# i-HamidZafar/Federated-Learning-with-MPI

Hardware: AMD Instinct MI355X
Metric: samples/sec/client + rounds-to-target-accuracy, MLP on income data at 1/2/4/8 clients (higher is better)
Workload: dtype bf16

## Files before the change

### fedmi/ops/csrc/fl_device.h

```cpp
#pragma once
#include "fl_common.h"
#include <math.h>


#define FL_STAMP(i)                                                                            \
    do {                                                                                       \
        if (b.dbg != nullptr && threadIdx.x == 0)                                              \
            b.dbg[blockIdx.x * 16 + (i)] = __builtin_amdgcn_s_memrealtime();                   \
    } while (0)

__device__ __forceinline__ void lds_barrier() { asm volatile("s_waitcnt lgkmcnt(0)\n\ts_barrier" ::: "memory"); }

__device__ __forceinline__ void lds_count_arrive(int* cnt) {
    asm volatile("s_waitcnt lgkmcnt(0)" ::: "memory");
    if ((threadIdx.x & 63) == 0) atomicAdd(cnt, 1);
}
__device__ __forceinline__ void lds_count_wait(int* cnt, int target) {
    while (*reinterpret_cast<volatile int*>(cnt) < target) __builtin_amdgcn_s_sleep(1);
    asm volatile("" ::: "memory");
}

__device__ __forceinline__ void slab_store(float* p, float v) {
#if defined(FL_SLAB_CACHED)
    *p = v;
#elif defined(FL_SLAB_NT)
    __builtin_nontemporal_store(v, p);
#else
    __hip_atomic_store(p, v, __ATOMIC_RELAXED, __HIP_MEMORY_SCOPE_AGENT);
#endif
}

__device__ __forceinline__ void slab_store_h(uint16_t* p, float v) {
    const float c = v == v ? fminf(fmaxf(v, -65504.f), 65504.f) : v;
    const _Float16 h = (_Float16)c;
#if defined(FL_SLAB_CACHED)
    *p = *reinterpret_cast<const uint16_t*>(&h);
#elif defined(FL_SLAB_NT)
    __builtin_nontemporal_store(*reinterpret_cast<const uint16_t*>(&h), p);
#else
    __hip_atomic_store(p, *reinterpret_cast<const uint16_t*>(&h), __ATOMIC_RELAXED, __HIP_MEMORY_SCOPE_AGENT);
#endif
}

__device__ __forceinline__ float wave_sum(float v) {
#pragma unroll
    for (int off = 32; off > 0; off >>= 1) v += __shfl_xor(v, off, 64);
    return v;
}

template <int THREADS>
__device__ __forceinline__ float block_sum_ordered(float acc, float* wsum) {
    acc = wave_sum(acc);
    if ((threadIdx.x & 63) == 0) wsum[threadIdx.x >> 6] = acc;
    __syncthreads();
    float ss = 0.f;
#pragma unroll
    for (int k = 0; k < THREADS / 64; ++k) ss = __fadd_rn(ss, wsum[k]);
    return ss;
}


template <typename CM>
__device__ void metrics_from_cm(CM cmv, int C, double out[4]) {
    double total = 0, tp_sum = 0;
    for (int t = 0; t < C; ++t)
        for (int p = 0; p < C; ++p) {
            const double x = cmv(t, p);
            total += x;
            if (t == p) tp_sum += x;
        }
    if (total <= 0) { out[0] = out[1] = out[2] = out[3] = 0; return; }
    double prec = 0, rec = 0, f1 = 0;
    for (int t = 0; t < C; ++t) {
        double support = 0, pred = 0;
        for (int p = 0; p < C; ++p) { support += cmv(t, p); pred += cmv(p, t); }
        const double tp = cmv(t, t);
        const double w = support / total;
        const double pc = pred > 0 ? tp / pred : 0.0;
        const double rc = support > 0 ? tp / support : 0.0;
        const double den = 2 * tp + (pred - tp) + (support - tp);
        const double fc = den > 0 ? 2 * tp / den : 0.0;
        prec += w * pc; rec += w * rc; f1 += w * fc;
    }
    out[0] = tp_sum / total; out[1] = prec; out[2] = rec; out[3] = f1;
}

static __device__ FLState fold_round(const MLPDesc& d, const FLConfig& c, const FLBuffers& b,
                                     const float* tails, int r, FLState S, bool write_hist) {
    const int lane = threadIdx.x & 63;
    if (S.stopped || r < 0 || r < S.finalized) return S;
    {
        const int C = d.dim[d.L];
        double mk[4] = {0, 0, 0, 0};
        double lk = 0;
        if (lane < c.world) {
            const float* cm = tails + lane * c.tail_stride;
            metrics_from_cm([&](int t, int p) { return (double)cm[t * C + p]; }, C, mk);
            lk = (double)cm[C * C];
            if (write_hist && r < c.max_rounds)
                for (int q = 0; q < 4; ++q) b.hist_rank[((size_t)r * c.world + lane) * 4 + q] = mk[q];
        }
        const float* rt = b.rtab + 4 * (size_t)r;
        const uint32_t m_lo = __float_as_uint(rt[2]), m_hi = __float_as_uint(rt[3]);
        const double n_act = (double)rt[1];
        auto sampled = [&](int k) { return ((k < 32 ? (m_lo >> k) : (m_hi >> (k - 32))) & 1u) != 0; };
        double mean[4] = {0, 0, 0, 0};
        double loss = 0;
        for (int k = 0; k < c.world; ++k) {
            const bool in = sampled(k);
            for (int q = 0; q < 4; ++q) {
                const double v = __shfl(mk[q], k, 64);
                if (in) mean[q] += v;
            }
            const double lv = __shfl(lk, k, 64);
            if (in) loss += lv;
        }
        if (lane != 0) return S;
        if (c.metric_mode == 0) {
            for (int q = 0; q < 4; ++q) mean[q] /= n_act;
        } else {
            metrics_from_cm(
                [&](int t, int p) {
                    double x = 0;
                    for (int k = 0; k < c.world; ++k)
// ... 44 lines not shown
```

### fedmi/ops/csrc/fl_kernels.hip

```cpp
#include "fl_common.h"
#include "fl_device.h"
#include "peer_device.h"
#include "fl_philox.h"
#include "fl_layout.h"
#include <math.h>

typedef float f32x4 __attribute__((ext_vector_type(4)));

__device__ __forceinline__ f32x4 mfma_f32(float a, float b, f32x4 c) {
    return __builtin_amdgcn_mfma_f32_16x16x4f32(a, b, c, 0, 0, 0);
}

__device__ __forceinline__ int fl_swz_lg(int lg) { return (lg == 1 || lg == 2) ? 4 : 0; }

__device__ __forceinline__ float4 lds4(const float* p) { return *reinterpret_cast<const float4*>(p); }
__device__ __forceinline__ float f4(const float4& v, int j) {
    return j == 0 ? v.x : (j == 1 ? v.y : (j == 2 ? v.z : v.w));
}

template <int RT, bool ST = false>
__device__ void fwd_layer_mfma(const float* w, int ldw, const float* bias, int K, int N, const float* in,
                               int ld_in, float* out, int ld_out, bool relu) {
    const int wave = threadIdx.x >> 6, lane = threadIdx.x & 63;
    const int lr = lane & 15, lg = lane >> 4;
    const int ntiles = (N + 15) >> 4;
    const int kchunks = (K + 15) >> 4;
    for (int nt = wave; nt < ntiles; nt += FL_WAVES) {
        const int n = nt * 16 + lr;
        const int ck = (4 * lg) ^ fl_swz(lr);
        const float* wr = w + n * ldw + ck;
        const float* ar = in + lr * ld_in + ck;
        f32x4 acc[RT];
#pragma unroll
        for (int rt = 0; rt < RT; ++rt) acc[rt] = (f32x4){0.f, 0.f, 0.f, 0.f};
        float4 bc = lds4(wr), ac[RT];
#pragma unroll
        for (int rt = 0; rt < RT; ++rt) ac[rt] = lds4(ar + rt * 16 * ld_in);
        const int klast = K - 16 * (kchunks - 1);
#pragma unroll ST ? 16 : 1
        for (int q = 0; q < kchunks; ++q) {
            const int qn = (q + 1 < kchunks) ? q + 1 : q;
            const float4 bn = lds4(wr + 16 * qn);
            float4 an[RT];
#pragma unroll
            for (int rt = 0; rt < RT; ++rt) an[rt] = lds4(ar + rt * 16 * ld_in + 16 * qn);
            __builtin_amdgcn_sched_barrier(0);
            const int jmax = (q + 1 < kchunks || klast > 4) ? 4 : klast;
#pragma unroll
            for (int j = 0; j < 4; ++j)
                if (j < jmax)
#pragma unroll
                    for (int rt = 0; rt < RT; ++rt) acc[rt] = mfma_f32(f4(ac[rt], j), f4(bc, j), acc[rt]);
            __builtin_amdgcn_sched_barrier(0);
            bc = bn;
#pragma unroll
            for (int rt = 0; rt < RT; ++rt) ac[rt] = an[rt];
        }
        const float bv = bias[n];
        const int ns = n ^ fl_swz_lg(lg);
#pragma unroll
        for (int rt = 0; rt < RT; ++rt)
#pragma unroll
            for (int j = 0; j < 4; ++j) {
                float v = acc[rt][j] + bv;
                if (relu) v = fmaxf(v, 0.f);
                out[(rt * 16 + lg * 4 + j) * ld_out + ns] = v;
            }
    }
}

template <int RT>
__device__ void fwd_head_valu(const float* w, int ldw, const float* bias, int K, int C, const float* in,
                              int ld_in, float* out, int ld_out) {
    const int R = RT * 16;
    const int nout = R * C;
    int T = FL_THREADS / nout;
    T = T >= 64 ? 64 : (T >= 32 ? 32 : (T >= 16 ? 16 : (T >= 8 ? 8 : (T >= 4 ? 4 : (T >= 2 ? 2 : 1)))));
    const int K16 = (K + 15) & ~15;
    for (int base = 0; base < nout * T; base += FL_THREADS) {
        const int gid = base + threadIdx.x;
        const int o = gid / T, part = gid - o * T;
        const int oc = o < nout ? o : nout - 1;
        const int r = oc / C, c = oc - r * C;
        const float* ar = in + r * ld_in;
        const float* wr = w + c * ldw;
        const int sa = fl_swz(r), sw = fl_swz(c);
        float s0 = 0.f, s1 = 0.f;
        int k = 4 * part;
        for (; k + 4 * T < K16; k += 8 * T) {
            const float4 a0 = lds4(ar + (k ^ sa)), w0 = lds4(wr + (k ^ sw));
            const float4 a1 = lds4(ar + ((k + 4 * T) ^ sa)), w1 = lds4(wr + ((k + 4 * T) ^ sw));
            s0 = fmaf(a0.x, w0.x, s0); s0 = fmaf(a0.y, w0.y, s0); s0 = fmaf(a0.z, w0.z, s0); s0 = fmaf(a0.w, w0.w, s0);
            s1 = fmaf(a1.x, w1.x, s1); s1 = fmaf(a1.y, w1.y, s1); s1 = fmaf(a1.z, w1.z, s1); s1 = fmaf(a1.w, w1.w, s1);
        }
        if (k < K16) {
            const float4 a0 = lds4(ar + (k ^ sa)), w0 = lds4(wr + (k ^ sw));
            s0 = fmaf(a0.x, w0.x, s0); s0 = fmaf(a0.y, w0.y, s0); s0 = fmaf(a0.z, w0.z, s0); s0 = fmaf(a0.w, w0.w, s0);
        }
        float s = s0 + s1;
        for (int off = 1; off < T; off <<= 1) s += __shfl_xor(s, off, 64);
        if (o < nout && part == 0) out[r * ld_out + (c ^ sa)] = s + bias[c];
    }
    const int Cp = (C + 15) & ~15;
    for (int e = threadIdx.x; e < R * (Cp - C); e += FL_THREADS) {
        const int r = e / (Cp - C), c = C + (e - r * (Cp - C));
        out[r * ld_out + (c ^ fl_swz(r))] = 0.f;
    }
}

__device__ __forceinline__ int wgrad_waves_fp32(int K, int N, int l) {
    const int items = l > 0 ? (K + 15) >> 4 : 0;
    const int chunks = (N + 15) >> 4;
    return (items > 0 && chunks >= 4 && 2 * items <= FL_WAVES) ? FL_WAVES - items : FL_WAVES;
}

template <int RT, bool ST = false>
__device__ void dgrad_layer(const float* w, int ldw, int K, int N, const float* dz, int ld_z, const float* act,
                            int ld_a, float* out) {
    const int wave = (FL_WAVES - 1) - (threadIdx.x >> 6), lane = threadIdx.x & 63;
    const int lr = lane & 15, lg = lane >> 4;
    const int itiles = (K + 15) >> 4;
    const int ochunks = (N + 15) >> 4;
    const bool prio = ochunks >= 4 && wave < itiles;
    if (prio) __builtin_amdgcn_s_setprio(2);
    for (int it = wave; it < itiles; it += FL_WAVES) {
        const int i = it * 16 + lr;
        const int is = i ^ fl_swz_lg(lg);
        const float* wc = w + 4 * lg * ldw + is;
        const float* ar = dz + lr * ld_z + ((4 * lg) ^ fl_swz(lr));
        f32x4 acc[RT];
#pragma unroll
        for (int rt = 0; rt < RT; ++rt) acc[rt] = (f32x4){0.f, 0.f, 0.f, 0.f};
        float bc[4];
        float4 ac[RT];
#pragma unroll
        for (int j = 0; j < 4; ++j) bc[j] = wc[j * ldw];
#pragma unroll
        for (int rt = 0; rt < RT; ++rt) ac[rt] = lds4(ar + rt * 16 * ld_z);
#pragma unroll ST ? 16 : 1
        for (int q = 0; q < ochunks; ++q) {
            const int qn = (q + 1 < ochunks) ? q + 1 : q;
            float bn[4];
            float4 an[RT];
#pragma unroll
            for (int j = 0; j < 4; ++j) bn[j] = wc[(16 * qn + j) * ldw];
#pragma unroll
            for (int rt = 0; rt < RT; ++rt) an[rt] = lds4(ar + rt * 16 * ld_z + 16 * qn);
            __builtin_amdgcn_sched_barrier(0);
#pragma unroll
            for (int j = 0; j < 4; ++j)
#pragma unroll
                for (int rt = 0; rt < RT; ++rt) acc[rt] = mfma_f32(f4(ac[rt], j), bc[j], acc[rt]);
            __builtin_amdgcn_sched_barrier(0);
#pragma unroll
            for (int j = 0; j < 4; ++j) bc[j] = bn[j];
#pragma unroll
            for (int rt = 0; rt < RT; ++rt) ac[rt] = an[rt];
        }
        const bool ivalid = i < K;
#pragma unroll
        for (int rt = 0; rt < RT; ++rt)
#pragma unroll
            for (int j = 0; j < 4; ++j) {
                const int o = (rt * 16 + lg * 4 + j) * ld_a + is;
                out[o] = (ivalid && act[o] > 0.f) ? acc[rt][j] : 0.f;
            }
    }
    if (prio) __builtin_amdgcn_s_setprio(0);
}

template <int RT>
__device__ void wgrad_layer(int K, int N, const float* dz, int ld_z, const float* act, int ld_a,
                            float* __restrict__ gW, float* __restrict__ gb, int nw = FL_WAVES, bool top = false) {
    const int wave = threadIdx.x >> 6, lane = threadIdx.x & 63;
    const int lr = lane & 15, lg = lane >> 4;
    const int otiles = (N + 15) >> 4, itiles = (K + 15) >> 4;
    const int ntile = otiles * itiles;
    const int w = top ? FL_WAVES - 1 - wave : wave;
    for (int t0 = w < nw ? w : ntile; t0 < ntile; t0 += 2 * nw) {
        const int t1raw = t0 + nw;
        const bool has1 = t1raw < ntile;
        const int t1 = has1 ? t1raw : t0;
        const int ot0 = t0 / itiles, it0 = t0 - ot0 * itiles;
        const int ot1 = t1 / itiles, it1 = t1 - ot1 * itiles;
        const int ls = lr ^ fl_swz_lg(lg);
        const float* ap0 = dz + 4 * lg * ld_z + ot0 * 16 + ls;
        const float* bp0 = act + 4 * lg * ld_a + it0 * 16 + ls;
        const float* ap1 = dz + 4 * lg * ld_z + ot1 * 16 + ls;
        const float* bp1 = act + 4 * lg * ld_a + it1 * 16 + ls;
        float a0[RT * 4], b0[RT * 4], a1[RT * 4], b1[RT * 4];
#pragma unroll
        for (int q = 0; q < RT; ++q)
#pragma unroll
            for (int j = 0; j < 4; ++j) {
                const int s = 4 * q + j;
                a0[s] = ap0[(16 * q + j) * ld_z]; b0[s] = bp0[(16 * q + j) * ld_a];
                a1[s] = ap1[(16 * q + j) * ld_z]; b1[s] = bp1[(16 * q + j) * ld_a];
            }
        __builtin_amdgcn_sched_barrier(0);
        f32x4 acc0 = (f32x4){0.f, 0.f, 0.f, 0.f}, acc1 = acc0;
        if (has1) {
#pragma unroll
            for (int s = 0; s < RT * 4; ++s) {
                acc0 = mfma_f32(a0[s], b0[s], acc0);
                acc1 = mfma_f32(a1[s], b1[s], acc1);
            }
        } else {
#pragma unroll
            for (int s = 0; s < RT * 4; ++s) acc0 = mfma_f32(a0[s], b0[s], acc0);
        }
        __builtin_amdgcn_sched_barrier(0);
        const int i0 = it0 * 16 + lr, i1 = it1 * 16 + lr;
#pragma unroll
        for (int j = 0; j < 4; ++j) {
            const int o0 = ot0 * 16 + lg * 4 + j, o1 = ot1 * 16 + lg * 4 + j;
            if (i0 < K && o0 < N) slab_store(&gW[o0 * K + i0], acc0[j]);
            if (has1 && i1 < K && o1 < N) slab_store(&gW[o1 * K + i1], acc1[j]);
        }
    }
    for (int o = threadIdx.x; o < N; o += FL_THREADS) {
        float s0 = 0.f, s1 = 0.f;
#pragma unroll
        for (int r = 0; r < RT * 16; r += 2) {
            s0 += dz[r * ld_z + (o ^ fl_swz(r))];
            s1 += dz[(r + 1) * ld_z + (o ^ fl_swz(r + 1))];
        }
        slab_store(&gb[o], s0 + s1);
    }
}

template <int RT>
__device__ void stage_rows(const float* __restrict__ X, int n_rows, int F, int row0, float* xs, int ld) {
    const int F16 = (F + 15) & ~15;
    for (int e = threadIdx.x; e < RT * 16 * ld; e += FL_THREADS) {
        const int r = e / ld, cs = e - r * ld;
        const int c = cs < F16 ? cs ^ fl_swz(r) : cs;
        const int row = row0 + r;
        const bool ok = row < n_rows && c < F;
        const float v = X[(size_t)(ok ? row : 0) * F + (ok ? c : 0)];
        xs[e] = ok ? v : 0.f;
    }
}

template <class SP = FlShapeDyn>
__device__ __forceinline__ void stage_image(const MLPDesc& d_, const float* __restrict__ params, float* li) {
    FL_SHAPE_D(SP, d, d_);
    const float4* src = reinterpret_cast<const float4*>(params);
    float4* dst = reinterpret_cast<float4*>(li);
    const int n4 = d.Pimg >> 2;
    for (int e = threadIdx.x; e < n4; e += FL_THREADS) dst[e] = src[e];
}

template <int RT, class SP = FlShapeDyn>
__device__ void forward_block(const MLPDesc& d_, float* acts, const float* li, unsigned long long* dbg = nullptr) {
    FL_SHAPE_D(SP, d, d_);
#pragma unroll SP::kStatic ? FL_MAX_LAYERS : 1
    for (int l = 0; l < d.L; ++l) {
        if (dbg != nullptr && threadIdx.x == 0) dbg[blockIdx.x * 16 + 10 + l] = __builtin_amdgcn_s_memrealtime();
        const int K = d.dim[l], N = d.dim[l + 1];
        const float* w = li + d.iw_off[l];
        const float* bias = li + d.ib_off[l];
        if (l + 1 == d.L && RT * 16 * N <= 128)
            fwd_head_valu<RT>(w, fl_ldw(K), bias, K, N, acts + d.act_off[l], d.ld[l], acts + d.act_off[l + 1],
                              d.ld[l + 1]);
        else
            fwd_layer_mfma<RT, SP::kStatic>(w, fl_ldw(K), bias, K, N, acts + d.act_off[l], d.ld[l], acts + d.act_off[l + 1],
                               d.ld[l + 1], l + 1 < d.L);
        lds_barrier();
    }
}

#ifndef FL_FP32_DEVICE_ONLY
template <int RT>
__global__ void __launch_bounds__(FL_THREADS)
fl_train_kernel(MLPDesc d, FLConfig c, FLBuffers b, const float* __restrict__ pg,
                const FLState* __restrict__ st_in, FLState* __restrict__ st_out, int local_step, int mode,
                float* __restrict__ cm_out, int fold_mask) {
    using SP = FlShapeDyn;
#include "fl_train_body.inc"
}

template <int RT>
__global__ void __launch_bounds__(FL_THREADS)
fl_train_batch_kernel(MLPDesc d, const FLTrialDesc* __restrict__ T, FLSel pg_sel, FLSel si_sel, FLSel so_sel,
                      int local_step, int mode, FLSel cm_sel, int fold_mask) {
    const FLTrialDesc& t = T[blockIdx.y];
    const FLConfig c = t.c;
    const FLBuffers b = t.b;
    const float* __restrict__ pg = reinterpret_cast<const float*>(fl_sel(t, pg_sel));
    const FLState* __restrict__ st_in = reinterpret_cast<const FLState*>(fl_sel(t, si_sel));
    FLState* __restrict__ st_out = reinterpret_cast<FLState*>(fl_sel(t, so_sel));
    float* __restrict__ cm_out = reinterpret_cast<float*>(fl_sel(t, cm_sel));
    using SP = FlShapeDyn;
#include "fl_train_body.inc"
// ... 392 lines not shown
```

### fedmi/ops/csrc/fl_kernels_bf16.hip

```cpp
#include "fl_common.h"
#include "fl_device.h"
#include "peer_device.h"
#include "fl_bf16.h"
#include "fl_layout.h"
#include <math.h>
#include <stdint.h>

typedef float f32x4 __attribute__((ext_vector_type(4)));
typedef short bf16x8 __attribute__((ext_vector_type(8)));
typedef short bf16x4 __attribute__((ext_vector_type(4)));
typedef __attribute__((address_space(3))) bf16x4* lds_bf16x4_ptr;

typedef __bf16 bf16x2_t __attribute__((ext_vector_type(2)));
__device__ __forceinline__ uint32_t cvt_pk_bf16(float a, float b) {
    const bf16x2_t v = {(__bf16)a, (__bf16)b};
    return __builtin_bit_cast(uint32_t, v);
}

__device__ __forceinline__ bf16x8 ld128(const char* p) { return *reinterpret_cast<const bf16x8*>(p); }

__device__ __forceinline__ bf16x4 ld_tr(const char* p) {
    return __builtin_amdgcn_ds_read_tr16_b64_v4i16((lds_bf16x4_ptr)(p));
}
__device__ __forceinline__ bf16x8 cat8(bf16x4 a, bf16x4 b) {
    return (bf16x8){a[0], a[1], a[2], a[3], b[0], b[1], b[2], b[3]};
}

__device__ __forceinline__ f32x4 mfma32(bf16x8 a, bf16x8 b, f32x4 c) {
    return __builtin_amdgcn_mfma_f32_16x16x32_bf16(a, b, c, 0, 0, 0);
}
__device__ __forceinline__ f32x4 mfma16(bf16x4 a, bf16x4 b, f32x4 c) {
    return __builtin_amdgcn_mfma_f32_16x16x16bf16_1k(a, b, c, 0, 0, 0);
}

__device__ __forceinline__ void fl_pack_bf16_body(const MLPDesc& d, const MLPDescB& e, const float* __restrict__ params,
                                                  char* __restrict__ out) {
    const int id = blockIdx.x * blockDim.x + threadIdx.x;
    const int total = e.item_base[d.L];
    if (id < total) {
        int l = 0;
#pragma unroll
        for (int q = 1; q < FL_MAX_LAYERS; ++q) l += (q < d.L && id >= e.item_base[q]) ? 1 : 0;
        const int loc = id - e.item_base[l];
        const int nch = e.kp[l] >> 3;
        const int n = loc / nch, ch = loc - n * nch;
        const int K16 = (d.dim[l] + 15) & ~15, N16 = (d.dim[l + 1] + 15) & ~15;
        const bool ok = n < N16 && 8 * ch < K16;
        uint4 v = make_uint4(0u, 0u, 0u, 0u), w = make_uint4(0u, 0u, 0u, 0u);
        if (ok) {
            const float4* src = reinterpret_cast<const float4*>(params + d.iw_off[l] + n * fl_ldw(d.dim[l]) + 8 * ch);
            const bool sw = fl_swz(n) != 0;
            const float4 p0 = sw ? src[1] : src[0], p1 = sw ? src[0] : src[1];
            v = make_uint4(pack_bf16x2(p0.x, p0.y), pack_bf16x2(p0.z, p0.w), pack_bf16x2(p1.x, p1.y),
                           pack_bf16x2(p1.z, p1.w));
            w = make_uint4(pack_lo_bf16x2(p0.x, p0.y), pack_lo_bf16x2(p0.z, p0.w), pack_lo_bf16x2(p1.x, p1.y),
                           pack_lo_bf16x2(p1.z, p1.w));
        }
        char* dst = out + e.w_off[l] - e.param_off + fl_wrow(n, e.ldw[l], e.wgap) + 16 * (ch ^ fl_wswz(n, e.wxor));
        *reinterpret_cast<uint4*>(dst) = v;
        *reinterpret_cast<uint4*>(dst + e.wlo_delta) = w;
        return;
    }
    int bid = id - total;
    for (int l = 0; l < d.L; ++l) {
        if (bid < e.kp[l + 1]) {
            const int N16 = (d.dim[l + 1] + 15) & ~15;
            reinterpret_cast<float*>(out + e.bias_off[l] - e.param_off)[bid] = bid < N16 ? params[d.ib_off[l] + bid] : 0.f;
            return;
        }
        bid -= e.kp[l + 1];
    }
}

#ifndef FL_BF16_DEVICE_ONLY
__global__ void fl_pack_bf16_kernel(MLPDesc d, MLPDescB e, const float* __restrict__ params, char* __restrict__ out) {
    fl_pack_bf16_body(d, e, params, out);
}

__global__ void fl_pack_bf16_batch_kernel(MLPDesc d, MLPDescB e, const FLTrialDesc* __restrict__ T, FLSel params,
                                          FLSel out) {
    const FLTrialDesc& t = T[blockIdx.y];
    fl_pack_bf16_body(d, e, reinterpret_cast<const float*>(fl_sel(t, params)), fl_sel(t, out));
}
#endif

#define STAGE_P_UNROLL 8
#define STAGE_X_UNROLL 2
// ... 146 lines not shown
            for (int rt = 0; rt < RT; ++rt) {
                av[rt] = ld128(act + aoff + rt * 16 * lda * 2 + ks * 64);
                al[rt] = ld128(alo + aoff + rt * 16 * lda * 2 + ks * 64);
            }
#pragma unroll
            for (int rt = 0; rt < RT; ++rt) {
                acc[rt] = mfma32(av[rt], bv, acc[rt]);
                acl[rt] = mfma32(al[rt], bv, acl[rt]);
                acl[rt] = mfma32(av[rt], bl, acl[rt]);
            }
        }
        const int n = nt * 16 + wc;
        const float b = bias[n];
        const bool odd = lg & 1;
        if (last) {
            float* z = reinterpret_cast<float*>(lds + e.logit_off);
#pragma unroll
            for (int rt = 0; rt < RT; ++rt)
#pragma unroll
                for (int t = 0; t < 4; ++t) {
                    const float v = odd ? acc[rt][(t + 1) & 3] + acl[rt][(t + 1) & 3] : acc[rt][t] + acl[rt][t];
                    z[(rt * 16 + fl_out_row(lg, t)) * FL_LOGIT_LD + n] = v + b;
                }
        } else {
            uint16_t* out = reinterpret_cast<uint16_t*>(lds + e.act_off[l + 1]);
            uint16_t* olo = reinterpret_cast<uint16_t*>(lds + e.alo_off[l + 1]);
            const int ldo = e.lda[l + 1];
#pragma unroll
            for (int rt = 0; rt < RT; ++rt)
#pragma unroll
                for (int t = 0; t < 4; t += 2) {
                    if constexpr (NWV == FL_WAVES && !PLAIN) {
#pragma unroll
                        for (int q = 0; q < 2; ++q) {
                            const int u = t + q;
                            const float z = odd ? acc[rt][(u + 1) & 3] + acl[rt][(u + 1) & 3] : acc[rt][u] + acl[rt][u];
                            const float v = fmaxf(z + b, 0.f);
                            const int o = (rt * 16 + fl_out_row(lg, u)) * ldo + n;
                            out[o] = (uint16_t)bf16_bits(v);
                            olo[o] = (uint16_t)lo_bits(v);
                        }
                        continue;
                    }
                    float v[2];
#pragma unroll
                    for (int q = 0; q < 2; ++q) {
                        const int u = t + q;
                        const float z = odd ? acc[rt][(u + 1) & 3] + acl[rt][(u + 1) & 3] : acc[rt][u] + acl[rt][u];
                        v[q] = fmaxf(z + b, 0.f);
                    }
                    const uint32_t h = cvt_pk_bf16(v[0], v[1]);
                    const int o0 = (rt * 16 + fl_out_row(lg, t)) * ldo + n, o1 = (rt * 16 + fl_out_row(lg, t + 1)) * ldo + n;
                    out[o0] = (uint16_t)h;
                    out[o1] = (uint16_t)(h >> 16);
                    if constexpr (!PLAIN) {
                        const uint32_t lo =
                            cvt_pk_bf16(v[0] - __uint_as_float(h << 16), v[1] - __uint_as_float(h & 0xffff0000u));
                        olo[o0] = (uint16_t)lo;
                        olo[o1] = (uint16_t)(lo >> 16);
                    }
                }
        }
    }
}

template <bool F16>
__device__ __forceinline__ void slab_put(float* slab, int idx, float v) {
    if (F16) slab_store_h(reinterpret_cast<uint16_t*>(slab) + idx, v);
    else slab_store(slab + idx, v);
}
template <int RT, bool F16, class SP = FlShapeDyn>
__device__ void wgrad_layer_bf16(const MLPDesc& d_, const MLPDescB& e_, int l, const char* lds, float* __restrict__ slab,
                                 int nw) {
    FL_SHAPE_D(SP, d, d_);
    FL_SHAPE_E(SP, e, e_);
    const int wave = threadIdx.x >> 6, lane = threadIdx.x & 63;
    const int lr = lane & 15, lg = lane >> 4, lq = lr >> 2, lp = lr & 3;
    const int K = d.dim[l], N = d.dim[l + 1];
    const int otiles = (N + 15) >> 4, itiles = (K + 15) >> 4;
    const int ldd = e.lda[l + 1], lda = e.lda[l];
    const char* D = lds + e.dlt_off[l + 1];
    const char* act = lds + e.act_off[l];
    const int t0 = nw == FL_WAVES ? wave : (wave < nw ? nw - 1 - wave : otiles * itiles);
    for (int t = t0; t < otiles * itiles; t += nw) {
        const int ot = t / itiles, it = t - ot * itiles;
        f32x4 acc = (f32x4){0.f, 0.f, 0.f, 0.f};
        if (RT >= 2) {
#pragma unroll
            for (int h = 0; h < RT / 2; ++h) {
                const int r0 = 32 * h + 4 * lg + lq;
                const char* pa = D + (r0 * ldd + ot * 16 + 4 * lp) * 2;
                const char* pb = act + (r0 * lda + it * 16 + 4 * lp) * 2;
                const bf16x8 a = cat8(ld_tr(pa), ld_tr(pa + 16 * ldd * 2));
                const bf16x8 b = cat8(ld_tr(pb), ld_tr(pb + 16 * lda * 2));
                acc = mfma32(a, b, acc);
            }
        } else {
            const int r0 = 4 * lg + lq;
            const bf16x4 a = ld_tr(D + (r0 * ldd + ot * 16 + 4 * lp) * 2);
            const bf16x4 b = ld_tr(act + (r0 * lda + it * 16 + 4 * lp) * 2);
            acc = mfma16(a, b, acc);
        }
        const int i = it * 16 + lr;
#pragma unroll
        for (int j = 0; j < 4; ++j) {
            const int o = ot * 16 + 4 * lg + j;
            if (i < K && o < N) slab_put<F16>(slab, d.w_off[l] + o * K + i, acc[j]);
        }
    }
    const uint16_t* Dh = reinterpret_cast<const uint16_t*>(D);
    for (int o = threadIdx.x; o < N; o += FL_THREADS) {
        float s0 = 0.f, s1 = 0.f;
#pragma unroll
        for (int r = 0; r < RT * 16; r += 2) {
            s0 += bf16_to_f32(Dh[r * ldd + o]);
            s1 += bf16_to_f32(Dh[(r + 1) * ldd + o]);
        }
        slab_put<F16>(slab, d.b_off[l] + o, s0 + s1);
    }
}

template <class SP = FlShapeDyn>
__device__ __forceinline__ int wgrad_waves_bf16(const MLPDescB& e_, int l) {
    FL_SHAPE_E(SP, e, e_);
    const int items = l > 0 ? (e.kp[l] >> 4) : 0;
    const int steps = e.kp[l + 1] >> 5;
    return (items > 0 && steps >= 4 && 2 * items <= FL_WAVES) ? FL_WAVES - items : FL_WAVES;
}

template <int RT, bool HWCVT = false, class SP = FlShapeDyn>
__device__ void dgrad_layer_bf16(const MLPDesc& d_, const MLPDescB& e_, int l, char* lds) {
    FL_SHAPE_D(SP, d, d_);
    FL_SHAPE_E(SP, e, e_);
    const int wave = (FL_WAVES - 1) - (threadIdx.x >> 6), lane = threadIdx.x & 63;
    const int lr = lane & 15, lg = lane >> 4, lq = lr >> 2, lp = lr & 3;
    const int itiles = e.kp[l] >> 4;
    const int osteps = e.kp[l + 1] >> 5;
    const int ldd = e.lda[l + 1], lda = e.lda[l], ldw = e.ldw[l];
    const char* Dn = lds + e.dlt_off[l + 1];
    const char* W = lds + e.w_off[l];
    const uint16_t* act = reinterpret_cast<const uint16_t*>(lds + e.act_off[l]);
    uint16_t* out = reinterpret_cast<uint16_t*>(lds + e.dlt_off[l]);
    for (int it = wave; it < itiles; it += FL_WAVES) {
        f32x4 acc[RT];
#pragma unroll
        for (int rt = 0; rt < RT; ++rt) acc[rt] = (f32x4){0.f, 0.f, 0.f, 0.f};
        const char* pw = W + fl_wrow(8 * lg + lq, ldw, e.wgap) + 32 * it + 16 * ((lp >> 1) ^ fl_wswz(8 * lg, e.wxor)) +
                         8 * (lp & 1);
        const char* pa = Dn + (lr * ldd + 8 * lg) * 2;
#pragma unroll SP::kStatic ? 8 : 1
        for (int os = 0; os < osteps; ++os) {
            const char* pwk = pw + os * (64 * ldw + 4 * e.wgap);
            const bf16x8 bv = cat8(ld_tr(pwk), ld_tr(pwk + 4 * ldw * 2));
            bf16x8 av[RT];
#pragma unroll
            for (int rt = 0; rt < RT; ++rt) av[rt] = ld128(pa + rt * 16 * ldd * 2 + os * 64);
#pragma unroll
            for (int rt = 0; rt < RT; ++rt) acc[rt] = mfma32(av[rt], bv, acc[rt]);
        }
        const int i = it * 16 + lr;
        const bool odd = lg & 1;
#pragma unroll
        for (int rt = 0; rt < RT; ++rt)
#pragma unroll
            for (int t = 0; t < 4; t += 2) {
                if constexpr (!HWCVT) {
#pragma unroll
                    for (int q = 0; q < 2; ++q) {
                        const int u = t + q;
                        const float g = odd ? acc[rt][(u + 1) & 3] : acc[rt][u];
                        const int o = (rt * 16 + fl_out_row(lg, u)) * lda + i;
                        out[o] = act[o] != 0 && !(act[o] & 0x8000u) ? (uint16_t)bf16_bits(g) : (uint16_t)0;
                    }
                    continue;
                }
                const float g0 = odd ? acc[rt][(t + 1) & 3] : acc[rt][t];
                const float g1 = odd ? acc[rt][(t + 2) & 3] : acc[rt][t + 1];
                const uint32_t h = cvt_pk_bf16(g0, g1);
                const int o0 = (rt * 16 + fl_out_row(lg, t)) * lda + i, o1 = (rt * 16 + fl_out_row(lg, t + 1)) * lda + i;
                out[o0] = act[o0] != 0 && !(act[o0] & 0x8000u) ? (uint16_t)h : (uint16_t)0;
                out[o1] = act[o1] != 0 && !(act[o1] & 0x8000u) ? (uint16_t)(h >> 16) : (uint16_t)0;
            }
    }
}

template <int RT, bool PART>
__device__ __forceinline__ void fwd_sync(int* cnt, int& tgt) {
    if constexpr (PART) {
        tgt += FL_WAVES - FL_LAG_SPR * RT;
        lds_count_arrive(cnt);
        lds_count_wait(cnt, tgt);
    } else {
        lds_barrier();
// ... 625 lines not shown
```

### fedmi/ops/csrc/fl_train_bf16_body.inc

```
    extern __shared__ __attribute__((aligned(16))) char lds[];
    __shared__ FLState S_sh;
    __shared__ int dgrad_done;
    __shared__ int fwd_done;
    __shared__ f32x4 lag_parts[(LAG == 2 || LAG == 3) ? RT * (FL_LAG_SPR - 1) * FL_LAG_PARTS * 16 : 1];
    __shared__ int lag_ready[(LAG == 2 || LAG == 3) ? RT : 1];
    if constexpr (LAG == 3) {
        if (mode == FL_EVAL_LAGGED && local_step == 0 && (int)blockIdx.x >= c.n_slabs) {
            score_block_bf16<RT>(d, e, c, b, st_in, cm_out, lds, lag_parts, lag_ready);
            return;
        }
    }
    constexpr int LAGT = LAG == 3 ? 0 : LAG;
    FL_STAMP(0);
    if (threadIdx.x == 0) {
        dgrad_done = 0;
        if constexpr (LAGT == 2) {
            fwd_done = 0;
            for (int i = 0; i < RT; ++i) lag_ready[i] = 0;
        }
    }
    int* cm_s = reinterpret_cast<int*>(lds + e.cm_off);
    const int C = d.dim[d.L];
    if (threadIdx.x < 64) {
        FLState S0 = *st_in;
// ... 92 lines not shown
    FL_STAMP(2);

    const float* z = reinterpret_cast<const float*>(lds + e.logit_off);
    uint16_t* DL = reinterpret_cast<uint16_t*>(lds + e.dlt_off[L]);
    const int ldL = e.lda[L];
    const bool score = cm_s[FL_CM_FLAG] != 0;
    float lossv = 0.f;
    if (threadIdx.x < R) {
        const int r = threadIdx.x, row = row0 + r;
        const float* zr = z + r * FL_LOGIT_LD;
        uint16_t* dr = DL + r * ldL;
        if (row < c.n_rows && C == 2) {
            const int y = ylab;
            const float z0 = zr[0], z1 = zr[1];
            const float mx = fmaxf(z0, z1);
            const int best = z1 > z0 ? 1 : 0;
            if (score) atomicAdd(&cm_s[y * 2 + best], 1);
            const float e0 = __expf(z0 - mx), e1 = __expf(z1 - mx);
            const float se = (0.f + e0) + e1;
            const float inv_se = 1.f / se;
            const float lse = mx + __logf(se);
            lossv = (lse - (y ? z1 : z0)) * c.inv_n;
            const float d0 = e0 * inv_se - (y == 0 ? 1.f : 0.f), d1 = e1 * inv_se - (y == 1 ? 1.f : 0.f);
            if constexpr (LAGT == 2) {
                *reinterpret_cast<uint32_t*>(dr) = cvt_pk_bf16(c.slab_f16 ? d0 : d0 * c.inv_n, c.slab_f16 ? d1 : d1 * c.inv_n);
            } else {
                dr[0] = (uint16_t)bf16_bits(c.slab_f16 ? d0 : d0 * c.inv_n);
                dr[1] = (uint16_t)bf16_bits(c.slab_f16 ? d1 : d1 * c.inv_n);
            }
        } else if (row < c.n_rows) {
            const int y = ylab;
            float mx = zr[0], bv = zr[0];
            int best = 0;
            for (int k = 1; k < C; ++k) {
                mx = fmaxf(mx, zr[k]);
                if (zr[k] > bv) { bv = zr[k]; best = k; }
            }
            if (score) atomicAdd(&cm_s[y * C + best], 1);
            float se = 0.f;
            for (int k = 0; k < C; ++k) se += __expf(zr[k] - mx);
            const float inv_se = 1.f / se;
            const float lse = mx + __logf(se);
            lossv = (lse - zr[y]) * c.inv_n;
            for (int k = 0; k < C; ++k) {
                const float p = __expf(zr[k] - mx) * inv_se;
                const float dk = p - (k == y ? 1.f : 0.f);
                dr[k] = (uint16_t)bf16_bits(c.slab_f16 ? dk : dk * c.inv_n);
            }
        } else {
            for (int k = 0; k < C; ++k) dr[k] = 0;
        }
    }
    if (threadIdx.x < 64) {
        lossv = wave_sum(lossv);
        if (threadIdx.x == 0) slab[d.P] = lossv;
    }
    lds_barrier();
    if (score || lagged)
        for (int i = threadIdx.x; i < C * C; i += FL_THREADS)
            if (cm_s[i]) atomicAdd(&cm_out[i], (float)cm_s[i]);
    FL_STAMP(3);

    int dgrad_target = 0;
#pragma unroll SP::kStatic ? FL_MAX_LAYERS : 1
    for (int l = L - 1; l >= 0; --l) {
        const int nw = wgrad_waves_bf16<SP>(e, l);
        if (c.slab_f16) wgrad_layer_bf16<RT, true, SP>(d, e, l, lds, slab, nw);
        else wgrad_layer_bf16<RT, false, SP>(d, e, l, lds, slab, nw);
#ifdef FL_STAMP_FINE
        if (l == L - 2) FL_STAMP(7);
        if (l == L - 1) FL_STAMP(14);
        if (l == L - 2 && b.dbg != nullptr && threadIdx.x == 64 * (FL_WAVES - 1))
            b.dbg[blockIdx.x * 16 + 11] = __builtin_amdgcn_s_memrealtime();
#endif
        if (l > 0) dgrad_layer_bf16<RT, LAGT == 2, SP>(d, e, l, lds);
#ifdef FL_STAMP_FINE
        if (l == L - 2) FL_STAMP(13);
        if (l == L - 2 && b.dbg != nullptr && threadIdx.x == 64 * (FL_WAVES - 1))
            b.dbg[blockIdx.x * 16 + 12] = __builtin_amdgcn_s_memrealtime();
#endif
        if (nw < FL_WAVES && l > 0) {
            dgrad_target += FL_WAVES - nw;
            if ((int)(threadIdx.x >> 6) >= nw) lds_count_arrive(&dgrad_done);
            lds_count_wait(&dgrad_done, dgrad_target);
        } else {
            lds_barrier();
        }
        FL_STAMP(4 + (L - 1 - l));
    }
    FL_STAMP(15);
```

### fedmi/ops/csrc/fl_train_body.inc

```
    extern __shared__ __attribute__((aligned(16))) float lds[];
    __shared__ FLState S_sh;
    __shared__ int dgrad_done;
    FL_STAMP(0);
    if (b.dbg != nullptr && threadIdx.x == 0) b.dbg[blockIdx.x * 16 + 13] = __builtin_amdgcn_s_memtime();
    int* cm_s = reinterpret_cast<int*>(lds + d.cm_off);
    const int C = d.dim[d.L];
    if (threadIdx.x == 0) dgrad_done = 0;
    if (threadIdx.x < 64) {
        FLState S0 = *st_in;
        if (local_step == 0) {
            if (mode == FL_EVAL_CLASSIC) {
                if (blockIdx.x == 0 || fold_may_stop(c, S0))
                    S0 = finalize_state(d, c, b, pg, S0, blockIdx.x == 0, fold_mask);
                if (threadIdx.x == 0) {
                    S0.live = (!S0.stopped && S0.next_round < c.max_rounds) ? 1 : 0;
                    if (S0.live) { S0.cur_round = S0.next_round; S0.next_round += 1; }
                    if (blockIdx.x == 0) *st_out = S0;
                }
            } else if (threadIdx.x == 0) {
                S0.live = (!S0.stopped && S0.next_round < c.max_rounds) ? 1 : 0;
            }
        }
        if (threadIdx.x == 0) {
            S_sh = S0;
            cm_s[FL_CM_FLAG] = (local_step == 0 && mode == FL_EVAL_FUSED && S0.next_round > S0.finalized) ? 1 : 0;
        }
    }
    for (int i = threadIdx.x; i < C * C; i += FL_THREADS) cm_s[i] = 0;
    const float* params = (local_step == 0) ? pg : b.local;
    const int R = RT * 16;
    const int row0 = blockIdx.x * R;
    const int L = d.L;
    float* acts = lds;
    float* li = lds + d.img_lds;
    const int ylab = (threadIdx.x < R) ? b.y[min(row0 + (int)threadIdx.x, c.n_rows - 1)] : 0;
    stage_image<SP>(d, params, li);
    stage_rows<RT>(b.X, c.n_rows, d.dim[0], row0, acts + d.act_off[0], d.ld[0]);
    lds_barrier();
    FL_STAMP(1);
    if (!S_sh.live) return;
    float* slab = b.slab + (size_t)blockIdx.x * c.slab_stride;
    forward_block<RT, SP>(d, acts, li, b.dbg);
    FL_STAMP(2);
    if (b.dbg != nullptr && threadIdx.x == 0) b.dbg[blockIdx.x * 16 + 14] = __builtin_amdgcn_s_memtime();

    float* z = acts + d.act_off[L];
    const int ldz = d.ld[L];
    const bool score = cm_s[FL_CM_FLAG] != 0;
    float lossv = 0.f;
    if (threadIdx.x < R) {
        const int r = threadIdx.x, row = row0 + r;
        float* zr = z + r * ldz;
        const int sr = fl_swz(r);
        if (row < c.n_rows && C == 2) {
            const int y = ylab;
            const float z0 = zr[sr], z1 = zr[1 ^ sr];
            const float mx = fmaxf(z0, z1);
            if (score) atomicAdd(&cm_s[y * 2 + (z1 > z0 ? 1 : 0)], 1);
            const float e0 = expf(z0 - mx), e1 = expf(z1 - mx);
            const float se = (0.f + e0) + e1;
            lossv = (mx + logf(se) - (y ? z1 : z0)) * c.inv_n;
            zr[sr] = (e0 / se - (y == 0 ? 1.f : 0.f)) * c.inv_n;
            zr[1 ^ sr] = (e1 / se - (y == 1 ? 1.f : 0.f)) * c.inv_n;
        } else if (row < c.n_rows) {
            const int y = ylab;
            float mx = zr[sr], bv = zr[sr];
            int best = 0;
            for (int k = 1; k < C; ++k) {
                mx = fmaxf(mx, zr[k ^ sr]);
                if (zr[k ^ sr] > bv) { bv = zr[k ^ sr]; best = k; }
            }
            if (score) atomicAdd(&cm_s[y * C + best], 1);
            float se = 0.f;
            for (int k = 0; k < C; ++k) se += expf(zr[k ^ sr] - mx);
            const float lse = mx + logf(se);
            lossv = (lse - zr[y ^ sr]) * c.inv_n;
            for (int k = 0; k < C; ++k) {
                const float p = expf(zr[k ^ sr] - mx) / se;
                zr[k ^ sr] = (p - (k == y ? 1.f : 0.f)) * c.inv_n;
            }
        } else {
            for (int k = 0; k < C; ++k) zr[k ^ sr] = 0.f;
        }
    }
    if (threadIdx.x < 64) {
        lossv = wave_sum(lossv);
        if (threadIdx.x == 0) slab[d.P] = lossv;
    }
    lds_barrier();
    if (score)
        for (int i = threadIdx.x; i < C * C; i += FL_THREADS)
            if (cm_s[i]) atomicAdd(&cm_out[i], (float)cm_s[i]);
    FL_STAMP(3);

    int dgrad_target = 0;
    bool from_top = false;
#pragma unroll SP::kStatic ? FL_MAX_LAYERS : 1
    for (int l = L - 1; l >= 0; --l) {
        const float* dz = (l == L - 1) ? acts + d.act_off[L] : acts + d.dlt_off[l + 1];
        const float* act = acts + d.act_off[l];
        const int nw = wgrad_waves_fp32(d.dim[l], d.dim[l + 1], l);
        wgrad_layer<RT>(d.dim[l], d.dim[l + 1], dz, d.ld[l + 1], act, d.ld[l], slab + d.w_off[l],
                        slab + d.b_off[l], nw, from_top && nw == FL_WAVES);
#ifdef FL_STAMP_FINE
        if (l == L - 2) FL_STAMP(7);
        if (l == L - 2 && b.dbg != nullptr && threadIdx.x == 64 * (FL_WAVES - 1))
            b.dbg[blockIdx.x * 16 + 11] = __builtin_amdgcn_s_memrealtime();
#endif
        if (l > 0)
            dgrad_layer<RT, SP::kStatic>(li + d.iw_off[l], fl_ldw(d.dim[l]), d.dim[l], d.dim[l + 1], dz, d.ld[l + 1], act,
                            d.ld[l], acts + d.dlt_off[l]);
#ifdef FL_STAMP_FINE
        if (l == L - 2 && b.dbg != nullptr && threadIdx.x == 64 * (FL_WAVES - 1))
            b.dbg[blockIdx.x * 16 + 12] = __builtin_amdgcn_s_memrealtime();
#endif
        if (nw < FL_WAVES && l > 0) {
            dgrad_target += FL_WAVES - nw;
            if ((int)(threadIdx.x >> 6) >= nw) lds_count_arrive(&dgrad_done);
            lds_count_wait(&dgrad_done, dgrad_target);
            from_top = true;
        } else {
            lds_barrier();
            from_top = false;
        }
        FL_STAMP(4 + (L - 1 - l));
    }
    FL_STAMP(15);
```

Baseline: 455.4 million.

## Store weight gradients to slab as vector runs via buffer stores

For static shapes, the wgrad MFMA operands are swapped so each lane holds four consecutive input-dim outputs. The lane then writes them to the gradient slab as one 64/128-bit buffer store instead of scattered scalar atomic stores. A vectorised bias path (behind FL_BIAS_VEC) and an LDS-address-space spin wait are also added. This cuts global store instruction count, at the cost of depending on alignment assumptions enforced by static_assert. For the bf16 kernel the run path only turns on with FL_BF16_SLAB_RUNS.

New measurement: 447.0 million. 1.8% lower.

```diff
diff --git a/fedmi/ops/csrc/fl_device.h b/fedmi/ops/csrc/fl_device.h
--- a/fedmi/ops/csrc/fl_device.h
+++ b/fedmi/ops/csrc/fl_device.h
@@ -17,6 +17,12 @@
 }
 __device__ __forceinline__ void lds_count_wait(int* cnt, int target) {
     while (*reinterpret_cast<volatile int*>(cnt) < target) __builtin_amdgcn_s_sleep(1);
+    asm volatile("" ::: "memory");
+}
+__device__ __forceinline__ void lds_count_wait_lds(int* cnt, int target) {
+    typedef __attribute__((address_space(3))) int lds_int_t;
+    volatile lds_int_t* p = (volatile lds_int_t*)cnt;
+    while (*p < target) __builtin_amdgcn_s_sleep(1);
     asm volatile("" ::: "memory");
 }
 
@@ -40,6 +46,51 @@
 #else
     __hip_atomic_store(p, *reinterpret_cast<const uint16_t*>(&h), __ATOMIC_RELAXED, __HIP_MEMORY_SCOPE_AGENT);
 #endif
+}
+
+#if defined(FL_SLAB_CACHED)
+#define FL_SLAB_ST_AUX 0
+#elif defined(FL_SLAB_NT)
+#define FL_SLAB_ST_AUX 2
+#else
+#define FL_SLAB_ST_AUX 16
+#endif
+#if defined(FL_SLAB_ELEMENT_STORES)
+constexpr bool kSlabRuns = false, kSlabRunsBf16 = false;
+#elif defined(FL_BF16_SLAB_RUNS)
+constexpr bool kSlabRuns = true, kSlabRunsBf16 = true;
+#else
+constexpr bool kSlabRuns = true, kSlabRunsBf16 = false;
+#endif
+typedef unsigned int fl_u32x2 __attribute__((ext_vector_type(2)));
+typedef unsigned int fl_u32x4 __attribute__((ext_vector_type(4)));
+__device__ __forceinline__ __amdgpu_buffer_rsrc_t slab_row_rsrc(float* slab_row, int row_bytes) {
+    return __builtin_amdgcn_make_buffer_rsrc(slab_row, (short)0, row_bytes, 0x00020000);
+}
+__device__ __forceinline__ uint32_t slab_h2(float a, float b) {
+    const float ca = a == a ? fminf(fmaxf(a, -65504.f), 65504.f) : a;
+    const float cb = b == b ? fminf(fmaxf(b, -65504.f), 65504.f) : b;
+    const _Float16 ha = (_Float16)ca, hb = (_Float16)cb;
+    return (uint32_t)*reinterpret_cast<const uint16_t*>(&ha) | ((uint32_t)*reinterpret_cast<const uint16_t*>(&hb) << 16);
+}
+__device__ __forceinline__ void slab_store_run_h(__amdgpu_buffer_rsrc_t rs, int first, int count, float v0, float v1,
+                                                 float v2, float v3) {
+    if (count >= 4) {
+        const fl_u32x2 w = {slab_h2(v0, v1), slab_h2(v2, v3)};
+        __builtin_amdgcn_raw_buffer_store_b64(w, rs, first * 2, 0, FL_SLAB_ST_AUX);
+    } else if (count >= 2) {
+        __builtin_amdgcn_raw_buffer_store_b32(slab_h2(v0, v1), rs, first * 2, 0, FL_SLAB_ST_AUX);
+    }
+}
+__device__ __forceinline__ void slab_store_run(__amdgpu_buffer_rsrc_t rs, int first, int count, float v0, float v1,
+                                               float v2, float v3) {
+    if (count >= 4) {
+        const fl_u32x4 w = {__float_as_uint(v0), __float_as_uint(v1), __float_as_uint(v2), __float_as_uint(v3)};
+        __builtin_amdgcn_raw_buffer_store_b128(w, rs, first * 4, 0, FL_SLAB_ST_AUX);
+    } else if (count >= 2) {
+        const fl_u32x2 w = {__float_as_uint(v0), __float_as_uint(v1)};
+        __builtin_amdgcn_raw_buffer_store_b64(w, rs, first * 4, 0, FL_SLAB_ST_AUX);
+    }
 }
 
 __device__ __forceinline__ float wave_sum(float v) {
diff --git a/fedmi/ops/csrc/fl_kernels.hip b/fedmi/ops/csrc/fl_kernels.hip
--- a/fedmi/ops/csrc/fl_kernels.hip
+++ b/fedmi/ops/csrc/fl_kernels.hip
@@ -3,6 +3,7 @@
 #include "peer_device.h"
 #include "fl_philox.h"
 #include "fl_layout.h"
+#include "fl_slab_map.h"
 #include <math.h>
 
 typedef float f32x4 __attribute__((ext_vector_type(4)));
@@ -169,9 +170,10 @@
     if (prio) __builtin_amdgcn_s_setprio(0);
 }
 
-template <int RT>
+template <int RT, class SP = FlShapeDyn>
 __device__ void wgrad_layer(int K, int N, const float* dz, int ld_z, const float* act, int ld_a,
-                            float* __restrict__ gW, float* __restrict__ gb, int nw = FL_WAVES, bool top = false) {
+                            float* __restrict__ gW, float* __restrict__ gb, int nw = FL_WAVES, bool top = false,
+                            [[maybe_unused]] int l = 0, [[maybe_unused]] float* slab_row = nullptr) {
     const int wave = threadIdx.x >> 6, lane = threadIdx.x & 63;
     const int lr = lane & 15, lg = lane >> 4;
     const int otiles = (N + 15) >> 4, itiles = (K + 15) >> 4;
@@ -202,14 +204,27 @@
         if (has1) {
 #pragma unroll
             for (int s = 0; s < RT * 4; ++s) {
-                acc0 = mfma_f32(a0[s], b0[s], acc0);
-                acc1 = mfma_f32(a1[s], b1[s], acc1);
+                acc0 = (SP::kStatic && kSlabRuns) ? mfma_f32(b0[s], a0[s], acc0) : mfma_f32(a0[s], b0[s], acc0);
+                acc1 = (SP::kStatic && kSlabRuns) ? mfma_f32(b1[s], a1[s], acc1) : mfma_f32(a1[s], b1[s], acc1);
             }
         } else {
 #pragma unroll
-            for (int s = 0; s < RT * 4; ++s) acc0 = mfma_f32(a0[s], b0[s], acc0);
+            for (int s = 0; s < RT * 4; ++s)
+                acc0 = (SP::kStatic && kSlabRuns) ? mfma_f32(b0[s], a0[s], acc0) : mfma_f32(a0[s], b0[s], acc0);
         }
         __builtin_amdgcn_sched_barrier(0);
+        if constexpr (SP::kStatic && kSlabRuns) {
+            constexpr MLPDesc dc = *SP::pd;
+            static_assert(fl_slab_runs_ok(dc), "runs of 4 or 2 floats, 8-byte aligned");
+            const __amdgpu_buffer_rsrc_t srow = slab_row_rsrc(slab_row, dc.P * 4);
+            const FlSlabRun r0 = fl_slab_run(dc, l, t0, lane);
+            slab_store_run(srow, r0.first, r0.count, acc0[0], acc0[1], acc0[2], acc0[3]);
+            if (has1) {
+                const FlSlabRun r1 = fl_slab_run(dc, l, t1, lane);
+                slab_store_run(srow, r1.first, r1.count, acc1[0], acc1[1], acc1[2], acc1[3]);
+            }
+            continue;
+        }
         const int i0 = it0 * 16 + lr, i1 = it1 * 16 + lr;
 #pragma unroll
         for (int j = 0; j < 4; ++j) {
diff --git a/fedmi/ops/csrc/fl_kernels_bf16.hip b/fedmi/ops/csrc/fl_kernels_bf16.hip
--- a/fedmi/ops/csrc/fl_kernels_bf16.hip
+++ b/fedmi/ops/csrc/fl_kernels_bf16.hip
@@ -3,6 +3,7 @@
 #include "peer_device.h"
 #include "fl_bf16.h"
 #include "fl_layout.h"
+#include "fl_slab_map.h"
 #include <math.h>
 #include <stdint.h>
 
@@ -315,6 +316,12 @@
     const char* D = lds + e.dlt_off[l + 1];
     const char* act = lds + e.act_off[l];
     const int t0 = nw == FL_WAVES ? wave : (wave < nw ? nw - 1 - wave : otiles * itiles);
+    constexpr bool RUNS = SP::kStatic && kSlabRunsBf16;
+    [[maybe_unused]] __amdgpu_buffer_rsrc_t srow;
+    if constexpr (RUNS) {
+        static_assert(!SP::kStatic || fl_slab_runs_ok(d_const), "runs of 4 or 2 elements, dword aligned");
+        srow = slab_row_rsrc(slab, d.P * (F16 ? 2 : 4));
+    }
     for (int t = t0; t < otiles * itiles; t += nw) {
         const int ot = t / itiles, it = t - ot * itiles;
         f32x4 acc = (f32x4){0.f, 0.f, 0.f, 0.f};
@@ -326,13 +333,19 @@
                 const char* pb = act + (r0 * lda + it * 16 + 4 * lp) * 2;
                 const bf16x8 a = cat8(ld_tr(pa), ld_tr(pa + 16 * ldd * 2));
                 const bf16x8 b = cat8(ld_tr(pb), ld_tr(pb + 16 * lda * 2));
-                acc = mfma32(a, b, acc);
+                acc = RUNS ? mfma32(b, a, acc) : mfma32(a, b, acc);
             }
         } else {
             const int r0 = 4 * lg + lq;
             const bf16x4 a = ld_tr(D + (r0 * ldd + ot * 16 + 4 * lp) * 2);
             const bf16x4 b = ld_tr(act + (r0 * lda + it * 16 + 4 * lp) * 2);
-            acc = mfma16(a, b, acc);
+            acc = RUNS ? mfma16(b, a, acc) : mfma16(a, b, acc);
+        }
+        if constexpr (RUNS) {
+            const FlSlabRun run = fl_slab_run(d, l, t, lane);
+            if (F16) slab_store_run_h(srow, run.first, run.count, acc[0], acc[1], acc[2], acc[3]);
+            else slab_store_run(srow, run.first, run.count, acc[0], acc[1], acc[2], acc[3]);
+            continue;
         }
         const int i = it * 16 + lr;
 #pragma unroll
@@ -342,6 +355,26 @@
         }
     }
     const uint16_t* Dh = reinterpret_cast<const uint16_t*>(D);
+#ifdef FL_BIAS_VEC
+    if constexpr (RUNS) {
+        for (int o4 = 4 * threadIdx.x; o4 < N; o4 += 4 * FL_THREADS) {
+            float s0[4] = {0.f, 0.f, 0.f, 0.f}, s1[4] = {0.f, 0.f, 0.f, 0.f};
+#pragma unroll
+            for (int r = 0; r < RT * 16; r += 2) {
+                const uint2 u0 = *reinterpret_cast<const uint2*>(Dh + r * ldd + o4);
+                const uint2 u1 = *reinterpret_cast<const uint2*>(Dh + (r + 1) * ldd + o4);
+                s0[0] += __uint_as_float(u0.x << 16); s0[1] += __uint_as_float(u0.x & 0xffff0000u);
+                s0[2] += __uint_as_float(u0.y << 16); s0[3] += __uint_as_float(u0.y & 0xffff0000u);
+                s1[0] += __uint_as_float(u1.x << 16); s1[1] += __uint_as_float(u1.x & 0xffff0000u);
+                s1[2] += __uint_as_float(u1.y << 16); s1[3] += __uint_as_float(u1.y & 0xffff0000u);
+            }
+            const int cnt = N - o4 < 4 ? N - o4 : 4;
+            if (F16) slab_store_run_h(srow, d.b_off[l] + o4, cnt, s0[0] + s1[0], s0[1] + s1[1], s0[2] + s1[2], s0[3] + s1[3]);
+            else slab_store_run(srow, d.b_off[l] + o4, cnt, s0[0] + s1[0], s0[1] + s1[1], s0[2] + s1[2], s0[3] + s1[3]);
+        }
+        return;
+    }
+#endif
     for (int o = threadIdx.x; o < N; o += FL_THREADS) {
         float s0 = 0.f, s1 = 0.f;
 #pragma unroll
diff --git a/fedmi/ops/csrc/fl_slab_map.h b/fedmi/ops/csrc/fl_slab_map.h
--- /dev/null
+++ b/fedmi/ops/csrc/fl_slab_map.h
@@ -0,0 +1,25 @@
+#pragma once
+#include "fl_common.h"
+
+struct FlSlabRun {
+    int first;
+    int count;
+};
+
+__host__ __device__ constexpr int fl_slab_tiles(const MLPDesc& d, int l) {
+    return ((d.dim[l + 1] + 15) >> 4) * ((d.dim[l] + 15) >> 4);
+}
+__host__ __device__ constexpr FlSlabRun fl_slab_run(const MLPDesc& d, int l, int tile, int lane) {
+    const int K = d.dim[l], N = d.dim[l + 1];
+    const int itiles = (K + 15) >> 4;
+    const int ot = tile / itiles, it = tile - ot * itiles;
+    const int o = ot * 16 + (lane & 15), i0 = it * 16 + 4 * (lane >> 4);
+    const int left = K - i0;
+    return {d.w_off[l] + o * K + i0, (o < N && left > 0) ? (left < 4 ? left : 4) : 0};
+}
+
+__host__ __device__ constexpr bool fl_slab_runs_ok(const MLPDesc& d) {
+    for (int l = 0; l < d.L; ++l)
+        if ((d.dim[l] & 1) || (d.w_off[l] & 1)) return false;
+    return true;
+}
diff --git a/fedmi/ops/csrc/fl_train_bf16_body.inc b/fedmi/ops/csrc/fl_train_bf16_body.inc
--- a/fedmi/ops/csrc/fl_train_bf16_body.inc
+++ b/fedmi/ops/csrc/fl_train_bf16_body.inc
@@ -198,7 +198,8 @@
         if (nw < FL_WAVES && l > 0) {
             dgrad_target += FL_WAVES - nw;
             if ((int)(threadIdx.x >> 6) >= nw) lds_count_arrive(&dgrad_done);
-            lds_count_wait(&dgrad_done, dgrad_target);
+            if constexpr (SP::kStatic && kSlabRunsBf16) lds_count_wait_lds(&dgrad_done, dgrad_target);
+            else lds_count_wait(&dgrad_done, dgrad_target);
         } else {
             lds_barrier();
         }
diff --git a/fedmi/ops/csrc/fl_train_body.inc b/fedmi/ops/csrc/fl_train_body.inc
--- a/fedmi/ops/csrc/fl_train_body.inc
+++ b/fedmi/ops/csrc/fl_train_body.inc
@@ -100,8 +100,8 @@
         const float* dz = (l == L - 1) ? acts + d.act_off[L] : acts + d.dlt_off[l + 1];
         const float* act = acts + d.act_off[l];
         const int nw = wgrad_waves_fp32(d.dim[l], d.dim[l + 1], l);
-        wgrad_layer<RT>(d.dim[l], d.dim[l + 1], dz, d.ld[l + 1], act, d.ld[l], slab + d.w_off[l],
-                        slab + d.b_off[l], nw, from_top && nw == FL_WAVES);
+        wgrad_layer<RT, SP>(d.dim[l], d.dim[l + 1], dz, d.ld[l + 1], act, d.ld[l], slab + d.w_off[l],
+                            slab + d.b_off[l], nw, from_top && nw == FL_WAVES, l, slab);
 #ifdef FL_STAMP_FINE
         if (l == L - 2) FL_STAMP(7);
         if (l == L - 2 && b.dbg != nullptr && threadIdx.x == 64 * (FL_WAVES - 1))
@@ -117,7 +117,8 @@
         if (nw < FL_WAVES && l > 0) {
             dgrad_target += FL_WAVES - nw;
             if ((int)(threadIdx.x >> 6) >= nw) lds_count_arrive(&dgrad_done);
-            lds_count_wait(&dgrad_done, dgrad_target);
+            if constexpr (SP::kStatic) lds_count_wait_lds(&dgrad_done, dgrad_target);
+            else lds_count_wait(&dgrad_done, dgrad_target);
             from_top = true;
         } else {
             lds_barrier();
```
